# Celeborn2BeAlive/optix-test-smallpt

Measured on AMD Instinct MI355X. Metric: Mega path-samples/sec at 1024x768, higher is better.
Workload: dtype f32

## Files before the change

### optix-test-smallpt_amd/csrc/spt_pool.hip

```cpp
#include "spt_device.h"
#include "spt_kernel.h"
#include "spt_share.h"

namespace spt {

constexpr uint32_t kEpsBias = 0x38D1B717u + 1u;
constexpr uint32_t kInfKeyP = 0x60AD78ECu - kEpsBias;
constexpr int kPoolBlock = 256;
constexpr uint32_t kNoTask = 0xFFFFFFFFu;
constexpr int kStackWords = 16;
constexpr int kMaxUnroll = 24;
#ifndef SPT_POOL_NARROW
#define SPT_POOL_NARROW 1
#endif
#ifndef SPT_POOL_TASK_LDS
#define SPT_POOL_TASK_LDS 1
#endif
constexpr bool kTaskLds = SPT_POOL_TASK_LDS != 0;
constexpr int kSlotBytes = kTaskLds ? 70 : 62;
constexpr int kSharePool = kTaskLds ? 144 : 160;

__device__ __forceinline__ uint32_t lane_id_p() { return __builtin_amdgcn_mbcnt_hi(~0u, __builtin_amdgcn_mbcnt_lo(~0u, 0u)); }
__device__ __forceinline__ uint32_t rank_in(unsigned long long m)
{
    return __builtin_amdgcn_mbcnt_hi((uint32_t)(m >> 32), __builtin_amdgcn_mbcnt_lo((uint32_t)m, 0u));
}
__device__ __forceinline__ unsigned long long lanes_where(bool p) { return __builtin_amdgcn_ballot_w64(p); }
__device__ __forceinline__ uint32_t wave_sum(uint32_t v)
{
    for (int off = 32; off > 0; off >>= 1) v += __shfl_down(v, off);
    return v;
}
__device__ __forceinline__ uint32_t uni(uint32_t v) { return __builtin_amdgcn_readfirstlane(v); }
__device__ __forceinline__ uint32_t umin2(uint32_t a, uint32_t b) { return a < b ? a : b; }
__device__ __forceinline__ uint32_t umin3(uint32_t a, uint32_t b, uint32_t c)
{
    uint32_t r;
    asm("v_min3_u32 %0, %1, %2, %3" : "=v"(r) : "v"(a), "v"(b), "v"(c));
    return r;
}

__device__ __forceinline__ uint32_t pack_path(uint32_t depth, uint32_t branchf, uint32_t inst, uint32_t refl, uint32_t sp)
{
    return depth | (branchf << 12) | (inst << 16) | (refl << 28) | (sp << 30);
}

enum { C_GEN = 0, C_DIFF = 1, C_REFR = 2 };

template <int P, int NG, int SH, bool OLD, typename... EP>
__device__ __forceinline__ void pool_body(const KParams& K, const EP&... env)
{
    constexpr bool ENV = kHasEnv<EP...>;
    static_assert(P % 16 == 0 && P <= 256, "pool size");
    extern __shared__ float4 lds[];
    constexpr int kWaveF4 = (kSlotBytes * P) / 16;
    static_assert((kSlotBytes * P) % 16 == 0, "wave region must be float4-aligned");
    const uint32_t lane = lane_id_p();
    const uint32_t wave = threadIdx.x >> 6;
    float4* const A0 = lds + wave * kWaveF4;
    float4* const A1 = A0 + P;
    float4* const A2 = A1 + P;
    float* const ACX = reinterpret_cast<float*>(A2 + P);
    float* const ACY = ACX + P;
    float* const ACZ = ACY + P;
    uint2* const TS = reinterpret_cast<uint2*>(ACZ + P);
    uint8_t* const LG = reinterpret_cast<uint8_t*>(ACZ + P) + (kTaskLds ? 8 * P : 0);
    float4* const s_geom = lds + (kPoolBlock / 64) * kWaveF4;
    float4* const s_mat = s_geom + 3 * NG;

    for (uint32_t i = threadIdx.x; i < 3u * NG; i += kPoolBlock) {
        const bool real = i < K.n;
        s_geom[i] = real ? K.geom[i] : make_float4(0.f, 0.f, 0.f, -__builtin_inff());
        s_mat[3 * i + 0] = real ? K.mat[3 * i + 0] : make_float4(0.f, 0.f, 0.f, 0.f);
        s_mat[3 * i + 1] = real ? K.mat[3 * i + 1] : make_float4(0.f, 0.f, 0.f, 0.f);
        s_mat[3 * i + 2] = real ? K.mat[3 * i + 2] : make_float4(0.f, 0.f, 0.f, 0.f);
    }
    if constexpr (ENV) {
        if (threadIdx.x == 0) { const EParams E = env_params(env...); s_mat[9 * NG] = make_float4(E.e[0], E.e[1], E.e[2], 0.f); }
    }
    const uint32_t wave_gid = blockIdx.x * (kPoolBlock / 64) + wave;
    uint2* const gtask = kTaskLds ? TS : K.slot_state + (size_t)wave_gid * P;
    for (uint32_t s = lane; s < (uint32_t)P; s += 64) {
        gtask[s] = make_uint2(kNoTask, 0u);
        A1[s].w = __uint_as_float(0u);
        LG[s] = (uint8_t)s;
    }
    __syncthreads();

    float4* const gstack = reinterpret_cast<float4*>(K.stack) + (size_t)wave_gid * (3 * 4 * P);
    auto stack_rec = [&](uint32_t e, uint32_t slot) -> float4* { return gstack + (slot * 3u + e) * 4u; };

    const f3 cam_o = mk(K.cam_o[0], K.cam_o[1], K.cam_o[2]);
    const f3 cam_d = mk(K.cam_d[0], K.cam_d[1], K.cam_d[2]);
    const f3 cam_cx = mk(K.cam_cx[0], K.cam_cx[1], K.cam_cx[2]);
    const f3 cam_cy = mk(K.cam_cy[0], K.cam_cy[1], K.cam_cy[2]);

    uint32_t nG = (uint32_t)P, nD = 0u, nR = 0u;
    uint32_t chunk_next = 0, chunk_end = 0;
    bool queue_empty = false;
    unsigned long long nbounce = 0;
    uint32_t nkill = 0;
    uint32_t nrec = 0;
    uint32_t itG = 0, itD = 0, itR = 0;
    uint32_t lnG = 0, lnD = 0, lnR = 0;
    uint32_t itTail = 0, itFull = 0;
    uint32_t lnTail = 0;
    uint32_t cntG = 0, cntD = 0, cntR = 0, cntDry = 0;
    const unsigned long long t_start = __builtin_amdgcn_s_memtime();
    uint32_t it_total = 0;
    bool timed_out = false;
    uint32_t dry_lo = 0, dry_hi = 0;
    uint32_t ord_lo, ord_hi, clk_lo, clk_hi, nch_v;
    asm volatile("v_mov_b32 %0, %5\n\tv_mov_b32 %1, %6\n\tv_mov_b32 %2, %7\n\tv_mov_b32 %3, %8\n\tv_mov_b32 %4, %9"
                 : "=v"(ord_lo), "=v"(ord_hi), "=v"(clk_lo), "=v"(clk_hi), "=v"(nch_v)
                 : "s"((uint32_t)(uintptr_t)K.chunk_order), "s"((uint32_t)((uintptr_t)K.chunk_order >> 32)),
                   "s"((uint32_t)(uintptr_t)K.chunk_clock), "s"((uint32_t)((uintptr_t)K.chunk_clock >> 32)), "s"(K.nchunks));

#ifdef SPT_POOL_PHASES
    unsigned long long ph[5] = {0, 0, 0, 0, 0};
#define PH_STAMP(i) { const unsigned long long t_ = __builtin_amdgcn_s_memtime(); ph[i] += t_ - ph_t; ph_t = t_; }
#else
#define PH_STAMP(i)
#endif
    for (;;) {
#ifdef SPT_POOL_PHASES
        unsigned long long ph_t = __builtin_amdgcn_s_memtime();
#endif
        uint32_t c, b, lbase;
        if (nR >= 64u) c = C_REFR;
        else if (nG >= 64u) c = C_GEN;
        else if (nD >= 64u) c = C_DIFF;
        else {
            c = C_DIFF;
            uint32_t m = nD;
            if (nG > m) { c = C_GEN; m = nG; }
            if (nR > m) { c = C_REFR; m = nR; }
            if (m == 0u) break;
        }
        if (c == C_GEN) { b = nG < 64u ? nG : 64u; nG -= b; lbase = nG; if constexpr (OLD) { ++itG; lnG += b; } }
        else if (c == C_DIFF) { b = nD < 64u ? nD : 64u; nD -= b; lbase = (uint32_t)P + nD; if constexpr (OLD) { ++itD; lnD += b; } }
        else { b = nR < 64u ? nR : 64u; lbase = 2u * (uint32_t)P - nR; nR -= b; if constexpr (OLD) { ++itR; lnR += b; } }
        if constexpr (OLD) {
            if (queue_empty) { ++itTail; lnTail += b; }
            if (b == 64u) ++itFull;
        }
        if ((++it_total & 255u) == 0u && K.watchdog_ticks != 0ull &&
            __builtin_amdgcn_s_memtime() - t_start > K.watchdog_ticks) { timed_out = true; break; }

        const bool valid = lane < b;
        const uint32_t slot = valid ? (uint32_t)LG[lbase + lane] : 0u;

        f3 o = mk(0, 0, 0), d = mk(0, 0, 1), w = mk(0, 0, 0);
        uint32_t depth = 0, branchf = 0, rbase = 0, k1 = 0, sp = 0;
        bool has_ray = false;
        bool retired = false;

        PH_STAMP(0)
        if (c == C_GEN) {
            if constexpr (!OLD) cntG += valid ? 1u : 0u;
            const uint2 ts = gtask[slot];
            uint32_t task = ts.x, snext = ts.y;
            sp = __float_as_uint(A1[slot].w) >> 30;
            uint32_t send = 0;
            if (task != kNoTask) {
                const uint32_t sbeg = (task & ((1u << K.nb_log2) - 1u)) * K.sb;
                send = sbeg + K.sb < K.samps ? sbeg + K.sb : K.samps;
            }
            bool gen = false;
            bool need_task = false;
            if (valid) {
                if (sp > 0u) {
                    --sp;
                    const float4* rec = stack_rec(sp, slot);
                    const float4 s0 = rec[0], s1 = rec[1], s2 = rec[2];
                    o = mk(s0.x, s0.y, s0.z); d = mk(s1.x, s1.y, s1.z); w = mk(s2.x, s2.y, s2.z);
                    const uint32_t db = __float_as_uint(s0.w);
                    depth = db & 0xFFFu; branchf = db >> 16;
                    const uint32_t k0 = __float_as_uint(s1.w);
                    k1 = __float_as_uint(s2.w);
                    rbase = rng_base(k0, branchf & 7u, depth);
                    has_ray = true;
                } else if (snext == send) {
                    need_task = true;
                } else {
                    gen = true;
                }
            }
            const unsigned long long need_mask = OLD ? __ballot(need_task) : lanes_where(need_task);
            if (need_mask != 0ull) {
                typedef __attribute__((address_space(1))) uint32_t* GWords;
                uint32_t c_lo = clk_lo, c_hi = clk_hi, o_lo = ord_lo, o_hi = ord_hi;
                asm volatile("" : "+v"(c_lo), "+v"(c_hi), "+v"(o_lo), "+v"(o_hi));
                const GWords clk = (GWords)(((unsigned long long)c_hi << 32) | c_lo);
                uint32_t now32;
                {
                    const unsigned long long t = __builtin_amdgcn_s_memtime();
                    asm volatile("v_mov_b32 %0, %1" : "=v"(now32) : "s"((uint32_t)(t >> 6)));
                }
                if (need_task && task != kNoTask) {
                    K.cells[task] = make_float4(ACX[slot], ACY[slot], ACZ[slot], 0.0f);
                    if (clk) (void)__hip_atomic_fetch_max(clk + nch_v + (task >> 6), now32, __ATOMIC_RELAXED, __HIP_MEMORY_SCOPE_AGENT);
                }
                const uint32_t cntn = (uint32_t)__popcll(need_mask);
                const uint32_t rk = rank_in(need_mask);
                const uint32_t avail = chunk_end - chunk_next;
                const uint32_t base_old = chunk_next;
                uint32_t base_new = 0;
                if (cntn > avail) {
                    if (!queue_empty) {
                        const int leader = __ffsll((long long)need_mask) - 1;
                        uint32_t nb = 0;
                        if ((int)lane == leader) nb = atomicAdd(K.queue, 64u);
                        base_new = uni(__shfl(nb, leader));
                        if (base_new >= K.ntasks) {
                            queue_empty = true;
                            const unsigned long long t = __builtin_amdgcn_s_memtime();
                            asm volatile("v_mov_b32 %0, %2\n\tv_mov_b32 %1, %3" : "=v"(dry_lo), "=v"(dry_hi) : "s"((uint32_t)t), "s"((uint32_t)(t >> 32)));
                            if constexpr (!OLD) cntDry = cntG + cntD + cntR;
                        } else {
                            const GWords ord = (GWords)(((unsigned long long)o_hi << 32) | o_lo);
                            if (ord) base_new = uni(ord[base_new >> 6]) << 6;
                            if (clk && (int)lane == leader) clk[base_new >> 6] = now32;
                        }
                    } else {
                        base_new = K.ntasks;
                    }
                    chunk_next = base_new + (cntn - avail);
                    chunk_end = base_new + 64u;
                    if (queue_empty) { chunk_next = chunk_end = 0; }
                } else {
                    chunk_next += cntn;
                }
                if (need_task) {
                    const uint32_t nt = rk < avail ? base_old + rk : base_new + (rk - avail);
                    if (nt < K.ntasks) {
                        task = nt; gen = true;
                        snext = (task & ((1u << K.nb_log2) - 1u)) * K.sb;
                        ACX[slot] = 0.f; ACY[slot] = 0.f; ACZ[slot] = 0.f;
                    } else {
                        retired = true;
                    }
                }
            }
            if (gen) {
                const uint32_t cellid = task >> K.nb_log2;
                const uint32_t pix_local = cellid >> 2, cell = cellid & 3u;
                const uint32_t ry = OLD ? pix_local / K.w : __umulhi(cellid >> 1, K.wdiv_mul) >> K.wdiv_shift;
                const uint32_t px = pix_local - ry * K.w;
                const uint32_t py = K.row_begin + (ry >> K.rb_log2) * K.rb_stride + (ry & K.rb_mask);
                const uint32_t pixel_idx = py * K.w + px;
                const uint32_t p0 = mix32(pixel_idx + K.s0);
                const uint32_t p1 = mix32(pixel_idx ^ K.s1);
                const uint32_t index_in_pixel = cell * K.samps + snext;
                const uint32_t k0 = mix32(p0 ^ (index_in_pixel * kGolden));
                k1 = mix32(p1 + index_in_pixel * 0x85EBCA6Bu);
                const float u1 = rng_draw(k0 + ((1u << 28) | 0u) * kGolden, k1);
                const float u2 = rng_draw(k0 + ((1u << 28) | 1u) * kGolden, k1);
                const uint32_t sx = cell & 1u, sy = cell >> 1;
                float ax, ay;
                if (K.sampler == 0u) {
                    const float r1 = 2 * u1;
                    const float q1 = sqrt_rsq(r1 < 1 ? r1 : 2 - r1);
                    const float dx = r1 < 1 ? q1 - 1 : 1 - q1;
                    const float r2 = 2 * u2;
                    const float q2 = sqrt_rsq(r2 < 1 ? r2 : 2 - r2);
                    const float dy = r2 < 1 ? q2 - 1 : 1 - q2;
                    const double tx = ((double)sx + .5 + (double)dx) / 2.0 + (double)px;
                    const double ty = ((double)sy + .5 + (double)dy) / 2.0 + (double)py;
                    const double qx0 = tx * K.inv_w, qy0 = ty * K.inv_h;
                    const double qx = __builtin_fma(__builtin_fma(-qx0, (double)K.w, tx), K.inv_w, qx0);
                    const double qy = __builtin_fma(__builtin_fma(-qy0, (double)K.h, ty), K.inv_h, qy0);
                    ax = (float)(qx - .5); ay = (float)(qy - .5);
                } else {
                    const float jx = ((float)sx + u1) * 0.5f, jy = ((float)sy + u2) * 0.5f;
                    const float fx = 0.5f * (2 * jx - 1), fy = 0.5f * (2 * jy - 1);
                    const float nx = (((float)px + 0.5f) + fx) * K.inv_wf;
                    const float ny = (((float)py + 0.5f) + fy) * K.inv_hf;
                    ax = 2.f * nx - 1.f; ay = 2.f * ny - 1.f;
                }
                const f3 dd = cam_cx * ax + cam_cy * ay + cam_d;
                const float inv = rcp_exact(sqrt_exact(dot(dd, dd)));
                o = cam_o + dd * K.cam_push;
                d = dd * inv;
                w = mk(1, 1, 1); depth = 0; branchf = 0; rbase = k0;
                gtask[slot] = make_uint2(task, snext + 1u);
                has_ray = true;
            }
        } else {
            const float4 a0 = A0[slot], a1 = A1[slot], a2 = A2[slot];
            const f3 hx = mk(a0.x, a0.y, a0.z);
            rbase = __float_as_uint(a0.w);
            const f3 din = mk(a1.x, a1.y, a1.z);
            const uint32_t pk = valid ? __float_as_uint(a1.w) : 0u;
            w = mk(a2.x, a2.y, a2.z);
            k1 = __float_as_uint(a2.w);
            depth = pk & 0xFFFu; branchf = (pk >> 12) & 0xFu; sp = pk >> 30;
            const uint32_t inst = (pk >> 16) & 0xFFFu;
            const float4 gh = s_geom[inst];
            const f3 n = normalize<false>(mk(hx.x - gh.x, hx.y - gh.y, hx.z - gh.z));
            const f3 nl = dot(n, din) < 0 ? n : neg(n);
            if (c == C_DIFF) {
                if constexpr (!OLD) cntD += valid ? 1u : 0u;
                const bool is_diff = valid && ((pk >> 28) & 3u) == 0u;
                o = hx + nl * 0.02f;
                if (is_diff) {
                    const uint32_t u1bits = rng_draw_bits(rbase + kGolden, k1);
                    const float r2 = rng_draw(rbase + 2u * kGolden, k1);
                    const float r2s = sqrt_rsq(r2);
                    float sn, cs;
                    sincos2pi_bits(u1bits, sn, cs);
                    const f3 ww = nl;
                    const bool ay = __builtin_fabsf(ww.x) >= 0.1f;
                    const f3 ur = mk(ay ? ww.z : 0.f, ay ? 0.f : -ww.z, ay ? -ww.x : ww.y);
                    const float s2 = ay ? ww.x : ww.y;
                    const float qu = ww.z * ww.z + s2 * s2;
                    const f3 uu = ur * rcp_exact<false>(sqrt_rsq<true, true>(qu));
                    const f3 vv = cross(ww, uu);
                    d = normalize<false>(uu * cs * r2s + vv * sn * r2s + ww * sqrt_rsq<true, true>(1 - r2));
                } else {
                    d = din - n * 2.0f * dot(n, din);
                }
                ++depth;
                rbase += 4u * kGolden;
                has_ray = valid;
            } else {
                if constexpr (!OLD) cntR += valid ? 1u : 0u;
                const float4 mfc = s_mat[3 * inst + (depth > 5u ? 2 : 1)];
                const f3 f = mk(mfc.x, mfc.y, mfc.z);
                const f3 off = nl * 0.02f;
                f3 no = hx + off, nf = f;
                f3 nd = din - n * 2.0f * dot(n, din);
                const bool into = dot(n, nl) > 0;
                const float nnt = into ? 1.0f / 1.5f : 1.5f / 1.0f;
                const float ddn = dot(din, nl);
                const float cos2t = 1 - nnt * nnt * (1 - ddn * ddn);
                if (valid && !(cos2t < 0)) {
                    const f3 tdir = normalize<true>(din * nnt - n * ((into ? 1.0f : -1.0f) * (ddn * nnt + sqrt_exact(cos2t))));
                    const float R0 = (0.5f * 0.5f) / (2.5f * 2.5f);
                    const float cc = 1 - (into ? -ddn : dot(tdir, n));
                    const float c2 = cc * cc;
                    const float Re = R0 + (1 - R0) * c2 * c2 * cc;
                    const float Tr = 1 - Re;
                    const f3 xin = hx - off;
                    if (depth <= 2u) {
                        const f3 tw = w * (f * Tr);
                        if (!(tw.x == 0.f && tw.y == 0.f && tw.z == 0.f)) {
                            const uint32_t br = branchf & 7u;
                            const bool nonfin = !(__builtin_fabsf(tw.x) < __builtin_inff() && __builtin_fabsf(tw.y) < __builtin_inff() && __builtin_fabsf(tw.z) < __builtin_inff());
                            float4* rec = stack_rec(sp, slot);
                            rec[0] = make_float4(xin.x, xin.y, xin.z, __uint_as_float((depth + 1u) | ((br | (1u << depth) | ((branchf & 8u) | (nonfin ? 8u : 0u))) << 16)));
                            rec[1] = make_float4(tdir.x, tdir.y, tdir.z, __uint_as_float(rbase - ((br << 29) | (depth << 2)) * kGolden));
                            rec[2] = make_float4(tw.x, tw.y, tw.z, __uint_as_float(k1));
                            rec[3] = make_float4(0.f, 0.f, 0.f, 0.f);
                            ++sp;
                            ++nrec;
                        }
                        nf = f * Re;
                    } else {
                        const float Pr = 0.25f + 0.5f * Re;
                        const bool pick_refl = rng_draw(rbase + kGolden, k1) < Pr;
                        const float inv = rcp_exact(pick_refl ? Pr : 1.f - Pr);
                        nf = f * (pick_refl ? Re : Tr) * inv;
                        if (!pick_refl) { no = xin; nd = tdir; }
                    }
                }
                w = w * nf;
                o = no; d = nd;
                ++depth;
                rbase += 4u * kGolden;
                if (valid) {
                    if (depth >= SPT_K_MAX_DEPTH) ++nkill;
                    else if (!(w.x == 0.f && w.y == 0.f && w.z == 0.f)) has_ray = true;
                    if (!(__builtin_fabsf(w.x) < __builtin_inff() && __builtin_fabsf(w.y) < __builtin_inff() && __builtin_fabsf(w.z) < __builtin_inff())) branchf |= 8u;
                }
            }
        }

        PH_STAMP(1)
        nbounce += (unsigned long long)__popcll(OLD ? __ballot(has_ray) : lanes_where(has_ray));
        uint32_t next = C_GEN;
        bool to_diff = false, to_refr = false;
        const bool queued = valid && !retired;
        uint32_t near_key = kInfKeyP, inst = 0;
        if (SPT_POOL_NARROW && 3 * NG <= 16 && b <= 4u) {
            const uint32_t r = lane >> 4, si = lane & 15u;
            const f3 ro = mk(__shfl(o.x, r), __shfl(o.y, r), __shfl(o.z, r));
            const f3 rd = mk(__shfl(d.x, r), __shfl(d.y, r), __shfl(d.z, r));
            uint32_t key = 0xFFFFFFFFu;
            if (si < 3u * NG) {
                const float4 g = s_geom[si];
                const f3 op = mk(g.x - ro.x, g.y - ro.y, g.z - ro.z);
                const float bb = dot(op, rd);
                const float det = bb * bb - dot(op, op) + g.w;
                const float sd = sqrt_rsq(det);
                const uint32_t key1 = __float_as_uint(bb - sd) - kEpsBias;
                const uint32_t key2 = __float_as_uint(bb + sd) - kEpsBias;
                key = key1 < key2 ? key1 : key2;
            }
            uint32_t m = key;
            m = umin2(m, (uint32_t)__builtin_amdgcn_update_dpp((int)m, (int)m, 0x121, 0xF, 0xF, false));
            m = umin2(m, (uint32_t)__builtin_amdgcn_update_dpp((int)m, (int)m, 0x122, 0xF, 0xF, false));
            m = umin2(m, (uint32_t)__builtin_amdgcn_update_dpp((int)m, (int)m, 0x124, 0xF, 0xF, false));
            m = umin2(m, (uint32_t)__builtin_amdgcn_update_dpp((int)m, (int)m, 0x128, 0xF, 0xF, false));
            const unsigned long long eq = __ballot(key == m);
            const uint32_t row = (uint32_t)(eq >> ((lane & 3u) * 16u)) & 0xFFFFu;
            const uint32_t m1 = (uint32_t)__builtin_amdgcn_readlane((int)m, 16), m2 = (uint32_t)__builtin_amdgcn_readlane((int)m, 32),
                           m3 = (uint32_t)__builtin_amdgcn_readlane((int)m, 48);
            const uint32_t mrow = lane == 1u ? m1 : (lane == 2u ? m2 : (lane == 3u ? m3 : m));
            if (has_ray) {
                near_key = mrow < kInfKeyP ? mrow : kInfKeyP;
                inst = (uint32_t)__ffs((int)row) - 1u;
            }
        } else if (has_ray) {
            uint32_t nk[3 * NG + 1];
            nk[0] = kInfKeyP;
            constexpr Share S = ShareOf<SH>::value;
            float opk[3 * NG][3], pd[3 * NG][3], pp[3 * NG][3], sd_xy[3 * NG], sp_xy[3 * NG];
#pragma unroll
            for (int base = 0; base < 3 * NG; base += 9) {
                float4 g[9];
#pragma unroll
                for (int j = 0; j < 9; ++j) {
                    if constexpr (SH == kShareNone) { if (base + j < 3 * NG) g[j] = s_geom[base + j]; }
                    else if (base + j < 3 * NG) {
                        typedef float v4f __attribute__((ext_vector_type(4)));
                        typedef __attribute__((address_space(3))) const volatile v4f* LdsV4;
                        const v4f v = *(LdsV4)(&s_geom[base + j]);
                        g[j] = make_float4(v.x, v.y, v.z, v.w);
                    }
                }
#pragma unroll
                for (int j = 0; j < 9; ++j) {
                    const int i = base + j;
                    if (i < 3 * NG && SH == kShareNone) {
                        const f3 op = mk(g[j].x - o.x, g[j].y - o.y, g[j].z - o.z);
                        const float bb = dot(op, d);
                        const float det = bb * bb - dot(op, op) + g[j].w;
                        const float sd = sqrt_rsq(det);
                        const uint32_t key1 = __float_as_uint(bb - sd) - kEpsBias;
                        const uint32_t key2 = __float_as_uint(bb + sd) - kEpsBias;
                        nk[i + 1] = umin3(nk[i], key1, key2);
                    } else if (i < 3 * NG) {
                        const float4 gj = g[j];
                        const float ok[3] = {o.x, o.y, o.z}, dk[3] = {d.x, d.y, d.z}, ck[3] = {gj.x, gj.y, gj.z};
#pragma unroll
                        for (int k = 0; k < 3; ++k) {
                            if (S.src[i][k] == i) {
                                opk[i][k] = ck[k] - ok[k];
                                pd[i][k] = opk[i][k] * dk[k];
                                pp[i][k] = opk[i][k] * opk[i][k];
                            }
                        }
                        const int ix = S.src[i][0], iy = S.src[i][1], iz = S.src[i][2], ixy = S.srcxy[i];
                        if (ixy == i) { sd_xy[i] = pd[ix][0] + pd[iy][1]; sp_xy[i] = pp[ix][0] + pp[iy][1]; }
                        const float bb = sd_xy[ixy] + pd[iz][2];
                        const float det = bb * bb - (sp_xy[ixy] + pp[iz][2]) + gj.w;
                        const float sd = sqrt_rsq(det);
                        const uint32_t key1 = __float_as_uint(bb - sd) - kEpsBias;
                        const uint32_t key2 = __float_as_uint(bb + sd) - kEpsBias;
                        nk[i + 1] = umin3(nk[i], key1, key2);
                    }
                }
            }
            near_key = nk[3 * NG];
#pragma unroll
            for (int i = 1; i < 3 * NG; ++i)
                if (nk[i + 1] != nk[i]) inst = (uint32_t)i;
        }
        PH_STAMP(2)
        if (has_ray) {
            if (near_key != kInfKeyP) {
                const float t = __uint_as_float(near_key + kEpsBias);
                const float4 me = s_mat[3 * inst + 0];
                const float4 mc = s_mat[3 * inst + 1];
                const float4 mf = s_mat[3 * inst + 2];
                const uint32_t rb = __float_as_uint(me.w);
                const uint32_t refl = rb & 3u;
                if ((rb & 4u) != 0u || (branchf & 8u) != 0u) {
                    ACX[slot] = ACX[slot] + w.x * me.x; ACY[slot] = ACY[slot] + w.y * me.y; ACZ[slot] = ACZ[slot] + w.z * me.z;
                }
                f3 f = mk(mc.x, mc.y, mc.z);
                bool cont = true;
                if (depth > 5u) {
                    if (rng_draw(rbase, k1) < mc.w) {
                        f = mk(mf.x, mf.y, mf.z);
                    } else {
                        cont = false;
                    }
                }
                if (cont) {
                    if (refl != 2u) {
                        w = w * f;
                        if (depth + 1u >= SPT_K_MAX_DEPTH) { ++nkill; cont = false; }
                        else if (w.x == 0.f && w.y == 0.f && w.z == 0.f) cont = false;
                    }
                    if (cont) {
                        const f3 hx = o + d * t;
                        A0[slot] = make_float4(hx.x, hx.y, hx.z, __uint_as_float(rbase));
                        A1[slot] = make_float4(d.x, d.y, d.z, __uint_as_float(pack_path(depth, branchf, inst, refl, sp)));
                        A2[slot] = make_float4(w.x, w.y, w.z, __uint_as_float(k1));
                        if constexpr (OLD) next = refl == 2u ? C_REFR : C_DIFF;
                        else { to_refr = refl == 2u; to_diff = !to_refr; }
                    }
                }
            } else if constexpr (ENV) {
                const float4 e = s_mat[9 * NG];
                ACX[slot] = ACX[slot] + w.x * e.x; ACY[slot] = ACY[slot] + w.y * e.y; ACZ[slot] = ACZ[slot] + w.z * e.z;
            }
        }
        PH_STAMP(3)
        if constexpr (!OLD) {
            const unsigned long long mq = lanes_where(queued), md = lanes_where(to_diff), mr = lanes_where(to_refr);
            const unsigned long long mg = mq & ~(md | mr);
            const bool to_gen = queued && !to_diff && !to_refr;
            uint32_t pos = nG + rank_in(mg);
            if (to_diff) pos = (uint32_t)P + nD + rank_in(md);
            if (to_refr) pos = 2u * (uint32_t)P - 1u - nR - rank_in(mr);
            if (queued) LG[pos] = (uint8_t)slot;
            if (to_gen) A1[slot].w = __uint_as_float(sp << 30);
            nG += (uint32_t)__popcll(mg);
            nD += (uint32_t)__popcll(md);
            nR += (uint32_t)__popcll(mr);
        } else {
            const bool to_gen = queued && next == C_GEN;
            const unsigned long long mg = __ballot(to_gen);
            const unsigned long long md = __ballot(queued && next == C_DIFF);
            const unsigned long long mr = __ballot(queued && next == C_REFR);
            uint32_t pos = nG + rank_in(mg);
            if (next == C_DIFF) pos = (uint32_t)P + nD + rank_in(md);
            if (next == C_REFR) pos = 2u * (uint32_t)P - 1u - nR - rank_in(mr);
            if (queued) LG[pos] = (uint8_t)slot;
            if (to_gen) A1[slot].w = __uint_as_float(sp << 30);
            nG += (uint32_t)__popcll(mg);
            nD += (uint32_t)__popcll(md);
            nR += (uint32_t)__popcll(mr);
        }
        PH_STAMP(4)
    }

    unsigned long long nk = nkill, nr = nrec;
    for (int off = 32; off > 0; off >>= 1) { nk += __shfl_down(nk, off); nr += __shfl_down(nr, off); }
    if constexpr (!OLD) {
        const uint32_t cnt = cntG + cntD + cntR, tail = queue_empty ? cnt - cntDry : 0u;
        itG = uni(cntG); itD = uni(cntD); itR = uni(cntR); itTail = uni(tail);
        itFull = (uint32_t)__builtin_amdgcn_readlane((int)cnt, 63);
        lnG = wave_sum(cntG); lnD = wave_sum(cntD); lnR = wave_sum(cntR); lnTail = wave_sum(tail);
    }
    if (lane == 0) {
        atomicAdd(&K.counters[0], nbounce);
        if (nk) atomicAdd(&K.counters[1], nk);
        atomicAdd(&K.counters[2], (unsigned long long)itG); atomicAdd(&K.counters[3], (unsigned long long)itD);
        atomicAdd(&K.counters[4], (unsigned long long)itR);
        atomicAdd(&K.counters[5], (unsigned long long)lnG); atomicAdd(&K.counters[6], (unsigned long long)lnD); atomicAdd(&K.counters[7], (unsigned long long)lnR);
        if (timed_out) atomicAdd(&K.counters[8], 1ull);
        atomicAdd(&K.counters[9], (unsigned long long)itTail); atomicAdd(&K.counters[10], (unsigned long long)lnTail);
        atomicAdd(&K.counters[11], (unsigned long long)itFull);
        const unsigned long long t_end = __builtin_amdgcn_s_memtime();
        atomicMax(&K.counters[12], t_end - t_start);
        const unsigned long long t_dry = ((unsigned long long)uni(dry_hi) << 32) | uni(dry_lo);
        if (t_dry) { atomicMax(&K.counters[13], t_end - t_dry); atomicAdd(&K.counters[14], t_end - t_dry); }
        atomicAdd(&K.counters[15], t_end - t_start);
#ifdef SPT_POOL_PHASES
        for (int i = 0; i < 5; ++i) atomicAdd(&K.counters[17 + i], ph[i]);
        atomicAdd(&K.counters[22], (unsigned long long)it_total);
#endif
        atomicAdd(&K.counters[16], nr);
    }
}

template <int P, int NG, int SH, typename... EP>
__global__ __launch_bounds__(kPoolBlock) void poolkernel(const KParams K, const EP... env) { pool_body<P, NG, SH, false, EP...>(K, env...); }
template <int P, int NG, int SH, typename... EP>
__global__ __launch_bounds__(kPoolBlock) void poolkernel_untrimmed(const KParams K, const EP... env) { pool_body<P, NG, SH, true, EP...>(K, env...); }

}

namespace spt {
__device__ __forceinline__ uint32_t cost_bucket(uint32_t cost)
{
    const uint32_t lg = 31u - (uint32_t)__builtin_clz(cost | 1u);
    const uint32_t frac = lg >= 3u ? (cost >> (lg - 3u)) & 7u : 0u;
    return 255u - (lg * 8u + frac);
}

constexpr uint32_t kOrderSlice = 4096;

__global__ __launch_bounds__(1024) void chunk_count_kernel(const uint32_t* __restrict__ clock, uint32_t n, uint32_t sorted, uint32_t* __restrict__ work)
{
    __shared__ uint32_t hist[256];
    if (threadIdx.x < 256u) hist[threadIdx.x] = 0u;
    __syncthreads();
    const uint32_t first = blockIdx.x * kOrderSlice, last = first + kOrderSlice < sorted ? first + kOrderSlice : sorted;
    for (uint32_t i = first + threadIdx.x; i < last; i += 1024u) atomicAdd(&hist[cost_bucket(clock[n + i] - clock[i])], 1u);
    __syncthreads();
    if (threadIdx.x < 256u && hist[threadIdx.x]) atomicAdd(&work[threadIdx.x], hist[threadIdx.x]);
}

__global__ __launch_bounds__(256) void chunk_scan_kernel(uint32_t* __restrict__ work)
{
    __shared__ uint32_t cnt[256];
    cnt[threadIdx.x] = work[threadIdx.x];
    __syncthreads();
    if (threadIdx.x == 0u) {
        uint32_t run = 0u;
        for (int b = 0; b < 256; ++b) { const uint32_t c = cnt[b]; cnt[b] = run; run += c; }
    }
    __syncthreads();
    work[256 + threadIdx.x] = cnt[threadIdx.x];
}

__global__ __launch_bounds__(1024) void chunk_scatter_kernel(const uint32_t* __restrict__ clock, uint32_t n, uint32_t sorted, uint32_t* __restrict__ work,
                                                             uint32_t* __restrict__ order)
{
    __shared__ uint32_t hist[256];
    if (threadIdx.x < 256u) hist[threadIdx.x] = 0u;
    __syncthreads();
    const uint32_t first = blockIdx.x * kOrderSlice, last = first + kOrderSlice < sorted ? first + kOrderSlice : sorted;
    for (uint32_t i = first + threadIdx.x; i < last; i += 1024u) atomicAdd(&hist[cost_bucket(clock[n + i] - clock[i])], 1u);
    __syncthreads();
    if (threadIdx.x < 256u) { const uint32_t c = hist[threadIdx.x]; hist[threadIdx.x] = c ? atomicAdd(&work[256 + threadIdx.x], c) : 0u; }
    __syncthreads();
    for (uint32_t i = first + threadIdx.x; i < last; i += 1024u) order[atomicAdd(&hist[cost_bucket(clock[n + i] - clock[i])], 1u)] = i;
    if (blockIdx.x == 0u) for (uint32_t i = sorted + threadIdx.x; i < n; i += 1024u) order[i] = i;
}
}

extern "C" hipError_t spt_pool_chunk_order(const uint32_t* chunk_clock, uint32_t nchunks, uint32_t ntasks, uint32_t* chunk_order, uint32_t* work512, hipStream_t stream)
{
    const uint32_t sorted = (ntasks & 63u) != 0u && nchunks > 0u ? nchunks - 1u : nchunks;
    const uint32_t slices = sorted ? (sorted + spt::kOrderSlice - 1u) / spt::kOrderSlice : 1u;
    hipError_t e = hipMemsetAsync(work512, 0, 256 * sizeof(uint32_t), stream);
    if (e != hipSuccess) return e;
    hipLaunchKernelGGL(spt::chunk_count_kernel, dim3(slices), dim3(1024), 0, stream, chunk_clock, nchunks, sorted, work512);
    hipLaunchKernelGGL(spt::chunk_scan_kernel, dim3(1), dim3(256), 0, stream, work512);
    hipLaunchKernelGGL(spt::chunk_scatter_kernel, dim3(slices), dim3(1024), 0, stream, chunk_clock, nchunks, sorted, work512, chunk_order);
    return hipGetLastError();
}

extern "C" size_t spt_pool_lds_bytes(uint32_t n, int pool)
{
    const uint32_t ng = n == 0 ? 1u : (n + 2u) / 3u;
    return (size_t)(spt::kPoolBlock / 64) * (size_t)spt::kSlotBytes * (size_t)pool + (size_t)ng * 3u * 64u;
}

extern "C" size_t spt_pool_stack_floats(uint32_t blocks, int pool)
{
    return (size_t)blocks * (spt::kPoolBlock / 64) * 3u * spt::kStackWords * (size_t)pool;
}

extern "C" size_t spt_pool_state_bytes(uint32_t blocks, int pool) { return (size_t)blocks * (spt::kPoolBlock / 64) * (size_t)pool * sizeof(uint2); }

extern "C" int spt_pool_max_spheres(void) { return spt::kMaxUnroll; }
extern "C" int spt_pool_default_slots(void) { return spt::kSharePool; }

template <int P, int NG, int SH, bool OLD, typename... EP>
static auto* pool_kernel_of()
{
    if constexpr (OLD) return &spt::poolkernel_untrimmed<P, NG, SH, EP...>;
    else return &spt::poolkernel<P, NG, SH, EP...>;
}

template <int P, int NG, int SH, bool OLD>
static hipError_t launch_pool(const spt::KParams* K, uint32_t blocks, size_t lds, hipStream_t stream, const float* env)
{
    if (env) {
        const spt::EParams E{{env[0], env[1], env[2]}};
        lds += 16u;
        auto* const kernel = pool_kernel_of<P, NG, SH, OLD, spt::EParams>();
        hipError_t e = hipFuncSetAttribute(reinterpret_cast<const void*>(kernel), hipFuncAttributeMaxDynamicSharedMemorySize, (int)lds);
        if (e != hipSuccess) return e;
        hipLaunchKernelGGL(kernel, dim3(blocks), dim3(spt::kPoolBlock), lds, stream, *K, E);
        return hipGetLastError();
    }
    auto* const kernel = pool_kernel_of<P, NG, SH, OLD>();
    hipError_t e = hipFuncSetAttribute(reinterpret_cast<const void*>(kernel), hipFuncAttributeMaxDynamicSharedMemorySize, (int)lds);
    if (e != hipSuccess) return e;
    hipLaunchKernelGGL(kernel, dim3(blocks), dim3(spt::kPoolBlock), lds, stream, *K);
    return hipGetLastError();
}

template <int P, int NG, bool OLD = false>
static hipError_t launch_pool_share(const spt::KParams* K, uint32_t blocks, size_t lds, hipStream_t stream, const float* env, int share)
{
    if constexpr (P == spt::kSharePool) {
        if constexpr (spt::share_compiled(spt::kShareCornell9, NG))
            if (share == spt::kShareCornell9) return launch_pool<P, NG, spt::kShareCornell9, OLD>(K, blocks, lds, stream, env);
        if constexpr (spt::share_compiled(spt::kShareBox, NG))
            if (share == spt::kShareBox) return launch_pool<P, NG, spt::kShareBox, OLD>(K, blocks, lds, stream, env);
    }
    if (share != spt::kShareNone) return hipErrorInvalidValue;
    return launch_pool<P, NG, spt::kShareNone, OLD>(K, blocks, lds, stream, env);
}

template <int P, bool OLD = false>
static hipError_t launch_pool_ng(const spt::KParams* K, uint32_t blocks, size_t lds, hipStream_t stream, const float* env, int share)
{
    switch (K->n == 0 ? 1u : (K->n + 2u) / 3u) {
    case 1: return launch_pool_share<P, 1, OLD>(K, blocks, lds, stream, env, share);
    case 2: return launch_pool_share<P, 2, OLD>(K, blocks, lds, stream, env, share);
    case 3: return launch_pool_share<P, 3, OLD>(K, blocks, lds, stream, env, share);
    case 4: return launch_pool_share<P, 4, OLD>(K, blocks, lds, stream, env, share);
    case 5: return launch_pool_share<P, 5, OLD>(K, blocks, lds, stream, env, share);
    case 6: return launch_pool_share<P, 6, OLD>(K, blocks, lds, stream, env, share);
    case 7: return launch_pool_share<P, 7, OLD>(K, blocks, lds, stream, env, share);
    case 8: return launch_pool_share<P, 8, OLD>(K, blocks, lds, stream, env, share);
    default: return hipErrorInvalidValue;
    }
}

extern "C" int spt_pool_has_size(int pool)
{
#ifdef SPT_POOL_SIZES
    if (pool == 96 || pool == 192) return 1;
#endif
    return pool == 128 || pool == 144 || pool == 160;
}

extern "C" int spt_pool_share_compiled(int pool, uint32_t n, int share)
{
    const int ng = n == 0 ? 1 : (int)((n + 2u) / 3u);
    return share == spt::kShareNone || (pool == spt::kSharePool && spt::share_compiled(share, ng));
}

extern "C" int spt_pool_has_old_loop(int pool) { return pool == spt::kSharePool; }

extern "C" hipError_t spt_pool_launch(const spt::KParams* K, uint32_t blocks, int pool, hipStream_t stream, const float* env, int share, int old_loop)
{
    const size_t lds = spt_pool_lds_bytes(K->n, pool);
    if (old_loop) return pool == spt::kSharePool ? launch_pool_ng<spt::kSharePool, true>(K, blocks, lds, stream, env, share) : hipErrorInvalidValue;
    if (pool == 128) return launch_pool_ng<128>(K, blocks, lds, stream, env, share);
    if (pool == 160) return launch_pool_ng<160>(K, blocks, lds, stream, env, share);
    if (pool == 144) return launch_pool_ng<144>(K, blocks, lds, stream, env, share);
#ifdef SPT_POOL_SIZES
    if (pool == 96) return launch_pool_ng<96>(K, blocks, lds, stream, env, share);
    if (pool == 192) return launch_pool_ng<192>(K, blocks, lds, stream, env, share);
#endif
    return hipErrorInvalidValue;
}
```

Measured before the change: 10810.

## Use wave-uniform lane masks for path control flow and repack path word

Adds a mask-based control path for the non-legacy, no-environment pool kernel. Per-lane booleans such as has_ray, need_task, gen, cont and the queue classification are replaced with 64-bit ballot masks and inverse_ballot tests, so compaction reuses masks instead of issuing fresh ballots. The packed path word is relaid out so the stack pointer, geometry byte offset and material offsets come out with a single mask and no shifts, and part of the packing is done early. The aim is fewer VALU and SALU instructions and less divergence handling in the hot bounce loop, at the cost of more code, inline asm and duplicated branches that could raise register pressure.

```diff
diff --git a/optix-test-smallpt_amd/csrc/spt_lanes.h b/optix-test-smallpt_amd/csrc/spt_lanes.h
--- /dev/null
+++ b/optix-test-smallpt_amd/csrc/spt_lanes.h
@@ -0,0 +1,12 @@
+#ifndef SPT_LANES_H
+#define SPT_LANES_H
+#include <stdint.h>
+#if defined(__HIPCC__)
+#define SPT_LANES_HD __host__ __device__ __forceinline__
+#else
+#define SPT_LANES_HD inline
+#endif
+
+SPT_LANES_HD uint64_t low_lanes(uint32_t b) { return b >= 64u ? ~(uint64_t)0 : ((uint64_t)1 << b) - 1u; }
+
+#endif
diff --git a/optix-test-smallpt_amd/csrc/spt_pool.hip b/optix-test-smallpt_amd/csrc/spt_pool.hip
--- a/optix-test-smallpt_amd/csrc/spt_pool.hip
+++ b/optix-test-smallpt_amd/csrc/spt_pool.hip
@@ -1,6 +1,7 @@
 #include "spt_device.h"
 #include "spt_kernel.h"
 #include "spt_share.h"
+#include "spt_lanes.h"
 
 namespace spt {
 
@@ -26,6 +27,10 @@
     return __builtin_amdgcn_mbcnt_hi((uint32_t)(m >> 32), __builtin_amdgcn_mbcnt_lo((uint32_t)m, 0u));
 }
 __device__ __forceinline__ unsigned long long lanes_where(bool p) { return __builtin_amdgcn_ballot_w64(p); }
+__device__ __forceinline__ bool lane_in(unsigned long long m) { return __builtin_amdgcn_inverse_ballot_w64(m); }
+__device__ __forceinline__ void bump(uint32_t& c) { asm volatile("v_add_u32 %0, 1, %0" : "+v"(c)); }
+__device__ __forceinline__ void pin(f3& v) { asm volatile("" : "+v"(v.x), "+v"(v.y), "+v"(v.z)); }
+__device__ __forceinline__ unsigned long long lanes_zero(const f3& v) { return lanes_where(v.x == 0.f) & lanes_where(v.y == 0.f) & lanes_where(v.z == 0.f); }
 __device__ __forceinline__ uint32_t wave_sum(uint32_t v)
 {
     for (int off = 32; off > 0; off >>= 1) v += __shfl_down(v, off);
@@ -45,12 +50,15 @@
     return depth | (branchf << 12) | (inst << 16) | (refl << 28) | (sp << 30);
 }
 
+constexpr uint32_t kSpShift = 15, kSpOne = 1u << kSpShift, kSpMask = 3u << kSpShift, kReflMask2 = 3u << 13, kGeomMask = 0x1FF0u;
+
 enum { C_GEN = 0, C_DIFF = 1, C_REFR = 2 };
 
 template <int P, int NG, int SH, bool OLD, typename... EP>
 __device__ __forceinline__ void pool_body(const KParams& K, const EP&... env)
 {
     constexpr bool ENV = kHasEnv<EP...>;
+    constexpr bool MASKS = !OLD && !ENV;
     static_assert(P % 16 == 0 && P <= 256, "pool size");
     extern __shared__ float4 lds[];
     constexpr int kWaveF4 = (kSlotBytes * P) / 16;
@@ -147,7 +155,9 @@
         if ((++it_total & 255u) == 0u && K.watchdog_ticks != 0ull &&
             __builtin_amdgcn_s_memtime() - t_start > K.watchdog_ticks) { timed_out = true; break; }
 
-        const bool valid = lane < b;
+        const unsigned long long vmask = low_lanes(b);
+        unsigned long long mh = 0ull, mret = 0ull;
+        const bool valid = OLD ? lane < b : lane_in(vmask);
         const uint32_t slot = valid ? (uint32_t)LG[lbase + lane] : 0u;
 
         f3 o = mk(0, 0, 0), d = mk(0, 0, 1), w = mk(0, 0, 0);
@@ -157,10 +167,9 @@
 
         PH_STAMP(0)
         if (c == C_GEN) {
-            if constexpr (!OLD) cntG += valid ? 1u : 0u;
             const uint2 ts = gtask[slot];
             uint32_t task = ts.x, snext = ts.y;
-            sp = __float_as_uint(A1[slot].w) >> 30;
+            sp = OLD ? __float_as_uint(A1[slot].w) >> 30 : __float_as_uint(A1[slot].w);
             uint32_t send = 0;
             if (task != kNoTask) {
                 const uint32_t sbeg = (task & ((1u << K.nb_log2) - 1u)) * K.sb;
@@ -168,25 +177,48 @@
             }
             bool gen = false;
             bool need_task = false;
-            if (valid) {
-                if (sp > 0u) {
-                    --sp;
-                    const float4* rec = stack_rec(sp, slot);
-                    const float4 s0 = rec[0], s1 = rec[1], s2 = rec[2];
-                    o = mk(s0.x, s0.y, s0.z); d = mk(s1.x, s1.y, s1.z); w = mk(s2.x, s2.y, s2.z);
-                    const uint32_t db = __float_as_uint(s0.w);
-                    depth = db & 0xFFFu; branchf = db >> 16;
-                    const uint32_t k0 = __float_as_uint(s1.w);
-                    k1 = __float_as_uint(s2.w);
-                    rbase = rng_base(k0, branchf & 7u, depth);
-                    has_ray = true;
-                } else if (snext == send) {
-                    need_task = true;
-                } else {
-                    gen = true;
-                }
-            }
-            const unsigned long long need_mask = OLD ? __ballot(need_task) : lanes_where(need_task);
+            unsigned long long mneed = 0ull, mgen = 0ull;
+            auto pop_child = [&]() {
+                sp -= kSpOne;
+                const float4* rec = stack_rec(sp >> kSpShift, slot);
+                const float4 s0 = rec[0], s1 = rec[1], s2 = rec[2];
+                o = mk(s0.x, s0.y, s0.z); d = mk(s1.x, s1.y, s1.z); w = mk(s2.x, s2.y, s2.z);
+                const uint32_t db = __float_as_uint(s0.w);
+                depth = db & 0xFFFu; branchf = db >> 16;
+                const uint32_t k0 = __float_as_uint(s1.w);
+                k1 = __float_as_uint(s2.w);
+                rbase = rng_base(k0, branchf & 7u, depth);
+            };
+            if constexpr (!MASKS) {
+                if constexpr (!OLD) { if (valid) bump(cntG); }
+                if (valid) {
+                    if (sp > 0u) {
+                        sp -= OLD ? 1u : kSpOne;
+                        const float4* rec = stack_rec(OLD ? sp : sp >> kSpShift, slot);
+                        const float4 s0 = rec[0], s1 = rec[1], s2 = rec[2];
+                        o = mk(s0.x, s0.y, s0.z); d = mk(s1.x, s1.y, s1.z); w = mk(s2.x, s2.y, s2.z);
+                        const uint32_t db = __float_as_uint(s0.w);
+                        depth = db & 0xFFFu; branchf = db >> 16;
+                        const uint32_t k0 = __float_as_uint(s1.w);
+                        k1 = __float_as_uint(s2.w);
+                        rbase = rng_base(k0, branchf & 7u, depth);
+                        has_ray = true;
+                    } else if (snext == send) {
+                        need_task = true;
+                    } else {
+                        gen = true;
+                    }
+                }
+            } else {
+                const unsigned long long mpop = vmask & lanes_where(sp != 0u);
+                mneed = vmask & ~mpop & lanes_where(snext == send);
+                mgen = vmask & ~(mpop | mneed);
+                mh = mpop;
+                if (valid) bump(cntG);
+                if (lane_in(mpop)) pop_child();
+                need_task = lane_in(mneed);
+            }
+            const unsigned long long need_mask = OLD ? __ballot(need_task) : (MASKS ? mneed : lanes_where(need_task));
             if (need_mask != 0ull) {
                 typedef __attribute__((address_space(1))) uint32_t* GWords;
                 uint32_t c_lo = clk_lo, c_hi = clk_hi, o_lo = ord_lo, o_hi = ord_hi;
@@ -231,18 +263,31 @@
                 } else {
                     chunk_next += cntn;
                 }
-                if (need_task) {
+                if constexpr (!MASKS) {
+                    if (need_task) {
+                        const uint32_t nt = rk < avail ? base_old + rk : base_new + (rk - avail);
+                        if (nt < K.ntasks) {
+                            task = nt; gen = true;
+                            snext = (task & ((1u << K.nb_log2) - 1u)) * K.sb;
+                            ACX[slot] = 0.f; ACY[slot] = 0.f; ACZ[slot] = 0.f;
+                        } else {
+                            retired = true;
+                        }
+                    }
+                } else {
                     const uint32_t nt = rk < avail ? base_old + rk : base_new + (rk - avail);
-                    if (nt < K.ntasks) {
-                        task = nt; gen = true;
+                    const unsigned long long mnew = need_mask & lanes_where(nt < K.ntasks);
+                    if (lane_in(mnew)) {
+                        task = nt;
                         snext = (task & ((1u << K.nb_log2) - 1u)) * K.sb;
                         ACX[slot] = 0.f; ACY[slot] = 0.f; ACZ[slot] = 0.f;
-                    } else {
-                        retired = true;
-                    }
-                }
-            }
-            if (gen) {
+                    }
+                    mgen |= mnew;
+                    mret = need_mask & ~mnew;
+                }
+            }
+            if constexpr (MASKS) mh |= mgen;
+            if (MASKS ? lane_in(mgen) : gen) {
                 const uint32_t cellid = task >> K.nb_log2;
                 const uint32_t pix_local = cellid >> 2, cell = cellid & 3u;
                 const uint32_t ry = OLD ? pix_local / K.w : __umulhi(cellid >> 1, K.wdiv_mul) >> K.wdiv_shift;
@@ -284,24 +329,25 @@
                 d = dd * inv;
                 w = mk(1, 1, 1); depth = 0; branchf = 0; rbase = k0;
                 gtask[slot] = make_uint2(task, snext + 1u);
-                has_ray = true;
+                if constexpr (!MASKS) has_ray = true;
             }
         } else {
             const float4 a0 = A0[slot], a1 = A1[slot], a2 = A2[slot];
             const f3 hx = mk(a0.x, a0.y, a0.z);
             rbase = __float_as_uint(a0.w);
             const f3 din = mk(a1.x, a1.y, a1.z);
-            const uint32_t pk = valid ? __float_as_uint(a1.w) : 0u;
+            const uint32_t pk = OLD ? (valid ? __float_as_uint(a1.w) : 0u) : __float_as_uint(a1.w);
             w = mk(a2.x, a2.y, a2.z);
             k1 = __float_as_uint(a2.w);
-            depth = pk & 0xFFFu; branchf = (pk >> 12) & 0xFu; sp = pk >> 30;
-            const uint32_t inst = (pk >> 16) & 0xFFFu;
-            const float4 gh = s_geom[inst];
+            if constexpr (OLD) { depth = pk & 0xFFFu; branchf = (pk >> 12) & 0xFu; sp = pk >> 30; }
+            else { depth = pk >> 20; branchf = pk & 0xFu; sp = pk & kSpMask; }
+            const uint32_t inst = OLD ? (pk >> 16) & 0xFFFu : pk & kGeomMask;
+            const float4 gh = OLD ? s_geom[inst] : *reinterpret_cast<const float4*>(reinterpret_cast<const char*>(s_geom) + inst);
             const f3 n = normalize<false>(mk(hx.x - gh.x, hx.y - gh.y, hx.z - gh.z));
             const f3 nl = dot(n, din) < 0 ? n : neg(n);
             if (c == C_DIFF) {
-                if constexpr (!OLD) cntD += valid ? 1u : 0u;
-                const bool is_diff = valid && ((pk >> 28) & 3u) == 0u;
+                if constexpr (!OLD) { if (valid) bump(cntD); }
+                const bool is_diff = valid && (OLD ? (pk >> 28) & 3u : pk & kReflMask2) == 0u;
                 o = hx + nl * 0.02f;
                 if (is_diff) {
                     const uint32_t u1bits = rng_draw_bits(rbase + kGolden, k1);
@@ -322,10 +368,11 @@
                 }
                 ++depth;
                 rbase += 4u * kGolden;
-                has_ray = valid;
+                if constexpr (!MASKS) has_ray = valid;
+                else mh = vmask;
             } else {
-                if constexpr (!OLD) cntR += valid ? 1u : 0u;
-                const float4 mfc = s_mat[3 * inst + (depth > 5u ? 2 : 1)];
+                const float4 mfc = OLD ? s_mat[3 * inst + (depth > 5u ? 2 : 1)]
+                                       : *reinterpret_cast<const float4*>(reinterpret_cast<const char*>(s_mat) + (3u * inst + (depth > 5u ? 32u : 16u)));
                 const f3 f = mk(mfc.x, mfc.y, mfc.z);
                 const f3 off = nl * 0.02f;
                 f3 no = hx + off, nf = f;
@@ -347,12 +394,12 @@
                         if (!(tw.x == 0.f && tw.y == 0.f && tw.z == 0.f)) {
                             const uint32_t br = branchf & 7u;
                             const bool nonfin = !(__builtin_fabsf(tw.x) < __builtin_inff() && __builtin_fabsf(tw.y) < __builtin_inff() && __builtin_fabsf(tw.z) < __builtin_inff());
-                            float4* rec = stack_rec(sp, slot);
+                            float4* rec = stack_rec(OLD ? sp : sp >> kSpShift, slot);
                             rec[0] = make_float4(xin.x, xin.y, xin.z, __uint_as_float((depth + 1u) | ((br | (1u << depth) | ((branchf & 8u) | (nonfin ? 8u : 0u))) << 16)));
                             rec[1] = make_float4(tdir.x, tdir.y, tdir.z, __uint_as_float(rbase - ((br << 29) | (depth << 2)) * kGolden));
                             rec[2] = make_float4(tw.x, tw.y, tw.z, __uint_as_float(k1));
                             rec[3] = make_float4(0.f, 0.f, 0.f, 0.f);
-                            ++sp;
+                            sp += OLD ? 1u : kSpOne;
                             ++nrec;
                         }
                         nf = f * Re;
@@ -368,21 +415,39 @@
                 o = no; d = nd;
                 ++depth;
                 rbase += 4u * kGolden;
-                if (valid) {
-                    if (depth >= SPT_K_MAX_DEPTH) ++nkill;
-                    else if (!(w.x == 0.f && w.y == 0.f && w.z == 0.f)) has_ray = true;
-                    if (!(__builtin_fabsf(w.x) < __builtin_inff() && __builtin_fabsf(w.y) < __builtin_inff() && __builtin_fabsf(w.z) < __builtin_inff())) branchf |= 8u;
+                if constexpr (!MASKS) {
+                    if (valid) {
+                        if constexpr (!OLD) bump(cntR);
+                        if (depth >= SPT_K_MAX_DEPTH) ++nkill;
+                        else if (!(w.x == 0.f && w.y == 0.f && w.z == 0.f)) has_ray = true;
+                        if (!(__builtin_fabsf(w.x) < __builtin_inff() && __builtin_fabsf(w.y) < __builtin_inff() && __builtin_fabsf(w.z) < __builtin_inff())) branchf |= 8u;
+                    }
+                } else {
+                    const unsigned long long mcap = vmask & lanes_where(depth >= SPT_K_MAX_DEPTH);
+                    mh = vmask & ~mcap & ~lanes_zero(w);
+                    if (lane_in(mcap)) bump(nkill);
+                    if (valid) {
+                        bump(cntR);
+                        if (!(__builtin_fabsf(w.x) < __builtin_inff() && __builtin_fabsf(w.y) < __builtin_inff() && __builtin_fabsf(w.z) < __builtin_inff())) branchf |= 8u;
+                    }
                 }
             }
         }
 
         PH_STAMP(1)
-        nbounce += (unsigned long long)__popcll(OLD ? __ballot(has_ray) : lanes_where(has_ray));
+        if constexpr (MASKS) has_ray = lane_in(mh);
+        uint32_t pre = 0u;
+        auto pack_class_part = [&]() {
+            if constexpr (MASKS) asm volatile("v_lshlrev_b32 %0, 20, %1\n\tv_or3_b32 %0, %0, %2, %3" : "=&v"(pre) : "v"(depth), "v"(branchf), "v"(sp));
+        };
+        nbounce += (unsigned long long)__popcll(OLD ? __ballot(has_ray) : (MASKS ? mh : lanes_where(has_ray)));
         uint32_t next = C_GEN;
         bool to_diff = false, to_refr = false;
         const bool queued = valid && !retired;
+        unsigned long long md = 0ull, mr = 0ull;
         uint32_t near_key = kInfKeyP, inst = 0;
-        if (SPT_POOL_NARROW && 3 * NG <= 16 && b <= 4u) {
+        pack_class_part();
+        if (SPT_POOL_NARROW && 3 * NG <= 16 && (MASKS ? __builtin_expect(b <= 4u, 0) : b <= 4u)) {
             const uint32_t r = lane >> 4, si = lane & 15u;
             const f3 ro = mk(__shfl(o.x, r), __shfl(o.y, r), __shfl(o.z, r));
             const f3 rd = mk(__shfl(d.x, r), __shfl(d.y, r), __shfl(d.z, r));
@@ -468,7 +533,41 @@
                 if (nk[i + 1] != nk[i]) inst = (uint32_t)i;
         }
         PH_STAMP(2)
-        if (has_ray) {
+        if constexpr (MASKS) {
+            const unsigned long long mhit = lanes_where(near_key != kInfKeyP);
+            if (mhit != 0ull) {
+                const float4 me = s_mat[3 * inst + 0];
+                const float4 mc = s_mat[3 * inst + 1];
+                const float4 mf = s_mat[3 * inst + 2];
+                const uint32_t rb = __float_as_uint(me.w);
+                const uint32_t refl = rb & 3u;
+                if (lane_in(mhit) && ((rb & 4u) != 0u || (branchf & 8u) != 0u)) {
+                    ACX[slot] = ACX[slot] + w.x * me.x; ACY[slot] = ACY[slot] + w.y * me.y; ACZ[slot] = ACZ[slot] + w.z * me.z;
+                }
+                f3 f = mk(mc.x, mc.y, mc.z);
+                unsigned long long mcont = mhit;
+                const unsigned long long mdeep = mhit & lanes_where(depth > 5u);
+                if (mdeep != 0ull) {
+                    mcont &= ~mdeep | lanes_where(rng_draw(rbase, k1) < mc.w);
+                    if (lane_in(mdeep)) { f = mk(mf.x, mf.y, mf.z); pin(f); }
+                }
+                const unsigned long long mrefr = lanes_where(refl == 2u);
+                const unsigned long long mext = mcont & ~mrefr;
+                if (lane_in(mext)) { w = w * f; pin(w); }
+                const unsigned long long mcap = mext & lanes_where(depth + 1u >= SPT_K_MAX_DEPTH);
+                if (lane_in(mcap)) bump(nkill);
+                mcont &= ~(mcap | (mext & lanes_zero(w)));
+                if (lane_in(mcont)) {
+                    const float t = __uint_as_float(near_key + kEpsBias);
+                    const f3 hx = o + d * t;
+                    A0[slot] = make_float4(hx.x, hx.y, hx.z, __uint_as_float(rbase));
+                    A1[slot] = make_float4(d.x, d.y, d.z, __uint_as_float(pre | (inst << 4) | (refl << 13)));
+                    A2[slot] = make_float4(w.x, w.y, w.z, __uint_as_float(k1));
+                }
+                md = mcont & ~mrefr;
+                mr = mcont & mrefr;
+            }
+        } else if (has_ray) {
             if (near_key != kInfKeyP) {
                 const float t = __uint_as_float(near_key + kEpsBias);
                 const float4 me = s_mat[3 * inst + 0];
@@ -497,7 +596,8 @@
                     if (cont) {
                         const f3 hx = o + d * t;
                         A0[slot] = make_float4(hx.x, hx.y, hx.z, __uint_as_float(rbase));
-                        A1[slot] = make_float4(d.x, d.y, d.z, __uint_as_float(pack_path(depth, branchf, inst, refl, sp)));
+                        A1[slot] = make_float4(d.x, d.y, d.z, __uint_as_float(OLD ? pack_path(depth, branchf, inst, refl, sp)
+                                                                                      : (depth << 20) | branchf | (inst << 4) | (refl << 13) | sp));
                         A2[slot] = make_float4(w.x, w.y, w.z, __uint_as_float(k1));
                         if constexpr (OLD) next = refl == 2u ? C_REFR : C_DIFF;
                         else { to_refr = refl == 2u; to_diff = !to_refr; }
@@ -509,18 +609,29 @@
             }
         }
         PH_STAMP(3)
-        if constexpr (!OLD) {
-            const unsigned long long mq = lanes_where(queued), md = lanes_where(to_diff), mr = lanes_where(to_refr);
+        if constexpr (MASKS) {
+            const unsigned long long mq = vmask & ~mret;
             const unsigned long long mg = mq & ~(md | mr);
-            const bool to_gen = queued && !to_diff && !to_refr;
             uint32_t pos = nG + rank_in(mg);
-            if (to_diff) pos = (uint32_t)P + nD + rank_in(md);
-            if (to_refr) pos = 2u * (uint32_t)P - 1u - nR - rank_in(mr);
-            if (queued) LG[pos] = (uint8_t)slot;
-            if (to_gen) A1[slot].w = __uint_as_float(sp << 30);
+            if (lane_in(md)) pos = (uint32_t)P + nD + rank_in(md);
+            if (lane_in(mr)) pos = 2u * (uint32_t)P - 1u - nR - rank_in(mr);
+            if (lane_in(mq)) LG[pos] = (uint8_t)slot;
+            if (lane_in(mg)) A1[slot].w = __uint_as_float(sp);
             nG += (uint32_t)__popcll(mg);
             nD += (uint32_t)__popcll(md);
             nR += (uint32_t)__popcll(mr);
+        } else if constexpr (!OLD) {
+            const unsigned long long mq = lanes_where(queued), mdp = lanes_where(to_diff), mrp = lanes_where(to_refr);
+            const unsigned long long mg = mq & ~(mdp | mrp);
+            const bool to_gen = queued && !to_diff && !to_refr;
+            uint32_t pos = nG + rank_in(mg);
+            if (to_diff) pos = (uint32_t)P + nD + rank_in(mdp);
+            if (to_refr) pos = 2u * (uint32_t)P - 1u - nR - rank_in(mrp);
+            if (queued) LG[pos] = (uint8_t)slot;
+            if (to_gen) A1[slot].w = __uint_as_float(sp);
+            nG += (uint32_t)__popcll(mg);
+            nD += (uint32_t)__popcll(mdp);
+            nR += (uint32_t)__popcll(mrp);
         } else {
             const bool to_gen = queued && next == C_GEN;
             const unsigned long long mg = __ballot(to_gen);
```

After: 11150, median of 6. +3.2%, better.
